# JdeRobot/slam-SDVL

Hardware: AMD Instinct MI355X
Metric: tracked frames/sec (640x480, 5-lvl pyr, ~200 feats) (higher is better)
Workload: dtype u8/f32/f64

## Files before the change

### include/sdvl_hip.h

```cpp
#ifndef SDVL_HIP_H_
#define SDVL_HIP_H_

#include <stdint.h>

#ifdef __cplusplus
extern "C" {
#endif

typedef struct sdvl_ctx sdvl_ctx;
typedef struct sdvl_frame sdvl_frame;

enum sdvl_status {
  SDVL_OK = 0,
  SDVL_ERR_INVALID = -1,
  SDVL_ERR_HIP = -2,
  SDVL_ERR_CAPACITY = -3,
  SDVL_ERR_NO_DEVICE = -4
};

#define SDVL_MAX_LEVELS 8
#define SDVL_MAX_CORNERS 6144
#define SDVL_MAX_ALIGN_FEATURES 2048
#define SDVL_CELL_KP_CAP 176
#define SDVL_MAX_CELL_SIZE 64
// ... 109 lines not shown
int sdvl_ctx_prefetch_images(sdvl_ctx *ctx, int n, const uint8_t *const *imgs, int stride, int width, int height, void *const *dev_dst);
int sdvl_ctx_prefetch_fence(sdvl_ctx *ctx, int ticket);
typedef struct sdvl_feed sdvl_feed;
int sdvl_feed_create(int device, int n_slots, sdvl_feed **out);
int sdvl_feed_destroy(sdvl_feed *f);
const char *sdvl_feed_last_error(const sdvl_feed *f);
int sdvl_feed_slot_arrived(sdvl_feed *f, int slot);
int sdvl_feed_images(sdvl_feed *f, int slot, int n, const uint8_t *const *imgs, int stride, int width, int height, void *const *dev_dst);
int sdvl_ctx_feed_acquire(sdvl_ctx *ctx, sdvl_feed *f, int slot);
int sdvl_ctx_feed_release(sdvl_ctx *ctx, sdvl_feed *f, int slot);
int sdvl_frame_set_image_device(sdvl_ctx *ctx, sdvl_frame *f, const void *dev_img, int stride);
int sdvl_frame_borrow_image_device(sdvl_ctx *ctx, sdvl_frame *f, const void *dev_img);
int sdvl_frames_own_images(sdvl_ctx *ctx, int n, sdvl_frame *const *frames);
int sdvl_pyramid_build(sdvl_ctx *ctx, int n, sdvl_frame *const *frames);
int sdvl_frame_download_level(sdvl_ctx *ctx, const sdvl_frame *f, int level, uint8_t *out, int stride);

int sdvl_fast_num_cells(int width, int height, const sdvl_detect_params *p, int *cells_per_level, int *total);
int sdvl_cell_kp_cap(int cell_size);
int64_t sdvl_detect_scratch_bytes(int width, int height, const sdvl_detect_params *p);
int sdvl_fast_cells(sdvl_ctx *ctx, int n, sdvl_frame *const *frames, const sdvl_detect_params *p, int cap,
                    sdvl_keypoint *out_kps, int32_t *out_cell_offsets);

int sdvl_detect_corners(sdvl_ctx *ctx, int n, sdvl_frame *const *frames, const sdvl_detect_params *p, int nfeatures);
int sdvl_frames_corner_counts(sdvl_ctx *ctx, int n, sdvl_frame *const *frames, int32_t *counts);
int sdvl_frame_download_corners(sdvl_ctx *ctx, sdvl_frame *f, int cap, int32_t *xyl, int *n_out);
int sdvl_retain_best(sdvl_ctx *ctx, uint32_t *packed, int len, int n_points, int cooperative, int *out_len);

int sdvl_frame_set_corners(sdvl_ctx *ctx, sdvl_frame *f, int n, const int32_t *xyl);
int sdvl_frames_set_corners(sdvl_ctx *ctx, int n, sdvl_frame *const *frames, const int32_t *counts, const int32_t *xyl);
int sdvl_frame_num_corners(const sdvl_frame *f);
int sdvl_frame_corner_capacity(const sdvl_frame *f);

int sdvl_shi_tomasi(sdvl_ctx *ctx, int n, sdvl_frame *const *frames, int cap, double *out_scores);

int sdvl_orb_describe(sdvl_ctx *ctx, int n, sdvl_frame *const *frames, int cap, uint8_t *out_desc);
int sdvl_frame_download_descriptors(sdvl_ctx *ctx, const sdvl_frame *f, int cap, uint8_t *out);
int sdvl_filter_inputs(sdvl_ctx *ctx, int n, sdvl_frame *const *frames, int cap, int32_t *xyl, double *scores, uint8_t *desc,
                       int32_t *counts);
int sdvl_filter_inputs_begin(sdvl_ctx *ctx, int n, sdvl_frame *const *frames, int cap, int with_desc);
int sdvl_filter_inputs_end(sdvl_ctx *ctx, int n, sdvl_frame *const *frames, int cap, int32_t *xyl, double *scores, uint8_t *desc,
                           int32_t *counts);
typedef struct sdvl_filtered_corner {
  int32_t index;
  int32_t x, y, level;
  int32_t score;
  int32_t pad_;
// ... 255 lines not shown
```

### slam-sdvl_amd/__init__.py

```python
import ctypes as C
import os

import numpy as np

try:
    import torch
except ImportError:
    torch = None

_HERE = os.path.dirname(os.path.abspath(__file__))
CSRC = os.path.join(_HERE, "csrc")
LIB_PATH = os.path.join(CSRC, "libsdvl_hip.so")
HOST_LIB_PATH = os.path.join(_HERE, "host", "libsdvl_host.so")

SDVL_GRAY8, SDVL_RGB8, SDVL_BGR8, SDVL_RGBA8, SDVL_BGRA8 = 0, 1, 2, 3, 4

MAX_LEVELS = 8
MAX_CORNERS = 6144

u8p = C.POINTER(C.c_uint8)
i32p = C.POINTER(C.c_int32)
f64p = C.POINTER(C.c_double)
f32p = C.POINTER(C.c_float)

# ... 68 lines not shown
class DepthParams(C.Structure):
    _fields_ = [("px_error_angle", C.c_double), ("min_depth", C.c_double), ("scale_min_dist", C.c_double),
                ("max_failed", C.c_int32), ("pad_", C.c_int32)]


class DepthOut(C.Structure):
    _fields_ = [("outcome", C.c_int32), ("n_failed", C.c_int32), ("rho", C.c_double), ("sigma2", C.c_double), ("a", C.c_double),
                ("b", C.c_double), ("cos_alpha", C.c_double), ("last_distance", C.c_double), ("position", C.c_double * 3)]


class SynthView(C.Structure):
    _fields_ = [("fx", C.c_double), ("fy", C.c_double), ("u0", C.c_double), ("v0", C.c_double),
                ("R", C.c_double * 9), ("t", C.c_double * 3), ("plane", C.c_double * 4),
                ("seed", C.c_uint32), ("frame_id", C.c_uint32), ("texture", C.c_uint32), ("reserved_", C.c_uint32),
                ("dist", C.c_double * 5)]


ABI_SYMBOLS = [
    "sdvl_ctx_create", "sdvl_ctx_destroy", "sdvl_last_error", "sdvl_ctx_synchronize", "sdvl_ctx_stream",
    "sdvl_ctx_bind_thread", "sdvl_ctx_device", "sdvl_pointer_device", "sdvl_ctx_scratch_device",
    "sdvl_ctx_timing_enable", "sdvl_ctx_timing_only", "sdvl_ctx_timing_get", "sdvl_ctx_timing_reset",
    "sdvl_frame_create", "sdvl_frame_create_many", "sdvl_frame_destroy", "sdvl_frame_upload", "sdvl_frames_upload", "sdvl_ctx_prefetch_images", "sdvl_ctx_prefetch_fence", "sdvl_frame_set_image_device", "sdvl_frame_borrow_image_device",
    "sdvl_pyramid_build", "sdvl_frame_download_level", "sdvl_fast_num_cells", "sdvl_cell_kp_cap", "sdvl_fast_cells",
    "sdvl_detect_corners", "sdvl_frames_corner_counts", "sdvl_frame_download_corners", "sdvl_retain_best",
    "sdvl_frame_set_corners", "sdvl_frames_set_corners", "sdvl_frame_num_corners", "sdvl_shi_tomasi", "sdvl_orb_describe",
    "sdvl_frame_download_descriptors", "sdvl_filter_inputs", "sdvl_filter_inputs_begin", "sdvl_filter_inputs_end", "sdvl_filter_corners_begin", "sdvl_filter_corners_end", "sdvl_orb_describe_points", "sdvl_hamming_argmin", "sdvl_image_align", "sdvl_image_align_begin", "sdvl_image_align_end", "sdvl_align_store_create", "sdvl_align_store_destroy", "sdvl_align_store_write", "sdvl_image_align_begin_stored", "sdvl_search_points", "sdvl_search_begin", "sdvl_search_slot", "sdvl_search_run", "sdvl_align_patches", "sdvl_pose_from_matches", "sdvl_search_points_filter", "sdvl_search_run_filter", "sdvl_search_run_chain", "sdvl_search_chain_end", "sdvl_frame_footprint", "sdvl_undistort", "sdvl_frames_upload_undistorted", "sdvl_convert_gray", "sdvl_frames_upload_color", "sdvl_ctx_set_wait_hook", "sdvl_ctx_wait_done", "sdvl_ctx_wait_block", "sdvl_ctx_health", "sdvl_ctx_counters",
    "sdvl_track_create", "sdvl_track_destroy", "sdvl_frame_register", "sdvl_frames_register", "sdvl_track_upload", "sdvl_track_append", "sdvl_track_align", "sdvl_track_search",
    "sdvl_track_collect", "sdvl_track_features", "sdvl_track_stats",
    "sdvl_synth_render", "sdvl_device_malloc", "sdvl_device_free", "sdvl_device_download",
    "sdvl_frames_own_images", "sdvl_feed_create", "sdvl_feed_destroy", "sdvl_feed_last_error", "sdvl_feed_slot_arrived", "sdvl_feed_images", "sdvl_ctx_feed_acquire", "sdvl_ctx_feed_release", "sdvl_frame_footprint_cap", "sdvl_ctx_set_corner_capacity", "sdvl_frame_corner_capacity", "sdvl_detect_scratch_bytes",
    "sdvl_ctx_set_wait_spin", "sdvl_ctx_fork_mark", "sdvl_ctx_fork_begin", "sdvl_ctx_fork_end", "sdvl_host_alloc_pinned", "sdvl_host_free_pinned", "sdvl_host_register", "sdvl_host_unregister",
]

_lib = None


def load_library():
    global _lib
    if _lib is None:
        if not os.path.exists(LIB_PATH):
            raise SdvlError("libsdvl_hip.so is not built (%s): run `python -c 'import __graft_entry__ as g; g.build()'`"
                            % LIB_PATH)
        lib = C.CDLL(LIB_PATH)
        lib.sdvl_last_error.restype = C.c_char_p
        lib.sdvl_last_error.argtypes = [C.c_void_p]
        lib.sdvl_ctx_stream.restype = C.c_void_p
        lib.sdvl_ctx_stream.argtypes = [C.c_void_p]
# ... 176 lines not shown

    def own_images(self, frames):
        arr = (C.c_void_p * len(frames))(*[f.h for f in frames])
        self._check(self.lib.sdvl_frames_own_images(self.h, len(frames), arr))

    def fast_cells(self, frames, dp, cap=None):
        n = len(frames)
        cpl = (C.c_int * 4)()
        tot = C.c_int()
        self._check(self.lib.sdvl_fast_num_cells(frames[0].width, frames[0].height, C.byref(dp), cpl, C.byref(tot)))
        if cap is None:
            cap = max(1, tot.value * self.lib.sdvl_cell_kp_cap(dp.cell_size))
        kps = (Keypoint * (n * cap))()
        offs = np.zeros((n, tot.value + 1), np.int32)
        arr = (C.c_void_p * n)(*[f.h for f in frames])
        self._check(self.lib.sdvl_fast_cells(self.h, n, arr, C.byref(dp), cap, kps, _ptr(offs, i32p)))
        raw = np.frombuffer(kps, dtype=np.dtype([("x", "<u2"), ("y", "<u2"), ("score", "u1"), ("level", "u1"), ("cell", "<u2")]))
        out = []
        for i in range(n):
            k = raw[i * cap: i * cap + offs[i, -1]]
            out.append((np.stack([k["x"], k["y"], k["score"], k["level"], k["cell"]], 1).astype(np.int32), offs[i].copy()))
        return out, [cpl[i] for i in range(dp.max_fast_levels)]

    def detect_corners(self, frames, dp, nfeatures=1000):
        n = len(frames)
        arr = (C.c_void_p * n)(*[f.h for f in frames])
        self._check(self.lib.sdvl_detect_corners(self.h, n, arr, C.byref(dp), nfeatures))
        counts = np.zeros(n, np.int32)
        self._check(self.lib.sdvl_frames_corner_counts(self.h, n, arr, _ptr(counts, i32p)))
        out = []
        for f, c in zip(frames, counts):
            xyl = np.zeros((max(int(c), 1), 3), np.int32)
            k = C.c_int()
            self._check(self.lib.sdvl_frame_download_corners(self.h, f.h, len(xyl), _ptr(xyl, i32p), C.byref(k)))
            out.append(xyl[:k.value].copy())
        return out

    def retain_best(self, packed, n_points, cooperative=0):
        packed = np.ascontiguousarray(packed, np.uint32).copy()
        k = C.c_int()
        self._check(self.lib.sdvl_retain_best(self.h, _ptr(packed, C.POINTER(C.c_uint32)), len(packed), int(n_points), int(cooperative),
                                              C.byref(k)))
        return packed[:k.value]

    def shi_tomasi(self, frames, cap=MAX_CORNERS):
        n = len(frames)
        out = np.zeros((n, cap), np.float64)
        arr = (C.c_void_p * n)(*[f.h for f in frames])
        self._check(self.lib.sdvl_shi_tomasi(self.h, n, arr, cap, _ptr(out, f64p)))
        return [out[i, :self.lib.sdvl_frame_num_corners(frames[i].h)].copy() for i in range(n)]
# ... 321 lines not shown
```

### slam-sdvl_amd/csrc/sdvl_detect.hip

```cpp
#include <atomic>

#include "sdvl_internal.h"
#include "sdvl_wave.h"

namespace {

constexpr int kPyrTW = 32, kPyrTH = 8;

struct PyrJob {
  const uint8_t *src;
  uint8_t *dst;
  int sw, sh, dw, dh;
};

__device__ __forceinline__ int reflect101_clamped(int p, int n) {
  if (p < 0) p = -p;
  if (p >= n) p = 2 * n - 2 - p;
  return min(max(p, 0), n - 1);
}

template <int kPyrTW, int kPyrTH>
__global__ __launch_bounds__(kPyrTW * kPyrTH / 4) void pyr_down_kernel(const PyrJob *__restrict__ jobs, int n_jobs, int gx, int gy) {
  constexpr int kThreads = kPyrTW * kPyrTH / 4;
  constexpr int kPyrSH = 2 * kPyrTH + 3;
  constexpr int kPyrSWW = kPyrTW / 2 + 2;
  constexpr int kPyrPitch = (kPyrSWW + 1) * 4;
  const auto sync = [] {
    if (kThreads == 64) wave_sync();
    else __syncthreads();
  };
  __shared__ uint32_t s_srcw[kPyrSH * (kPyrSWW + 1)];
  __shared__ __attribute__((aligned(8))) uint16_t s_h[kPyrSH][kPyrTW];
  const int id = blockIdx.x, per_frame = gx * gy;
  const int slot = id >> 3;
  const int bz = (slot / per_frame) * 8 + (id & 7);
  if (bz >= n_jobs) return;
  const int tq = slot % per_frame;
  const int by = tq / gx, bx = tq - by * gx;
  const PyrJob job = jobs[bz];
  const int tx0 = bx * kPyrTW, ty0 = by * kPyrTH;
  if (tx0 >= job.dw || ty0 >= job.dh) return;
// ... 32 lines not shown
      const int sy = reflect101_clamped(2 * ty0 - 2 + r, job.sh);
      const int wi = min(max(w0 + c, 0), words_row - 1);
      s_srcw[r * (kPyrSWW + 1) + c] = reinterpret_cast<const uint32_t *>(job.src + static_cast<size_t>(sy) * job.sw)[wi];
    }
    sync();
    if (tid < rows && (xb < 0 || xb + last_byte >= job.sw)) {
      uint8_t *row = s_bytes + tid * kPyrPitch;
      if (xb < 0) {
        row[2] = row[6];
        row[3] = row[5];
      }
      for (int b = max(2, job.sw - xb); b <= last_byte; b++) row[b] = row[max(reflect101_clamped(xb + b, job.sw) - xb, 0)];
    }
  } else {
    const int ncols = last_byte - 1;
    for (int idx = tid; idx < rows * ncols; idx += kThreads) {
      const int r = idx / ncols, c = idx - r * ncols;
      const int sy = reflect101_clamped(2 * ty0 - 2 + r, job.sh);
      const int sx = reflect101_clamped(2 * tx0 - 2 + c, job.sw);
      s_bytes[r * kPyrPitch + 2 + c] = job.src[static_cast<size_t>(sy) * job.sw + sx];
    }
  }
  sync();
  typedef unsigned short u16x2 __attribute__((ext_vector_type(2)));
  for (int idx = tid; idx < rows * (kPyrTW / 2); idx += kThreads) {
    const int r = idx / (kPyrTW / 2), xp = idx - r * (kPyrTW / 2);
    if (2 * xp < nx) {
      const uint32_t *w = &s_srcw[r * (kPyrSWW + 1) + xp];
      const uint32_t w0 = w[0], w1 = w[1], w2 = w[2];
      const uint32_t hx = __builtin_amdgcn_udot4(w1, 0x00010406u, __builtin_amdgcn_udot4(w0, 0x04010000u, 0u, false), false);
      const uint32_t hx1 = __builtin_amdgcn_udot4(w2, 0x00000001u, __builtin_amdgcn_udot4(w1, 0x04060401u, 0u, false), false);
      const uint32_t h = hx | (hx1 << 16);
      *reinterpret_cast<uint32_t *>(&s_h[r][2 * xp]) = __builtin_bit_cast(uint32_t, h);
    }
  }
  sync();
  {
    const int y = tid / (kPyrTW / 4), x = (tid % (kPyrTW / 4)) * 4;
    const int oy = ty0 + y, ox = tx0 + x;
    if (oy < job.dh && ox < job.dw) {
      u16x2 a01 = {0, 0}, a23 = {0, 0};
#pragma unroll
      for (int t = 0; t < 5; t++) {
        const unsigned short wg = (t == 0 || t == 4) ? 1 : (t == 2 ? 6 : 4);
        const u16x2 wgt = {wg, wg};
        const uint2 hv = *reinterpret_cast<const uint2 *>(&s_h[2 * y + t][x]);
        a01 += wgt * __builtin_bit_cast(u16x2, hv.x);
        a23 += wgt * __builtin_bit_cast(u16x2, hv.y);
      }
      const u16x2 half = {128, 128};
      a01 = (a01 + half) >> 8;
      a23 = (a23 + half) >> 8;
      int acc[4] = {a01.x, a01.y, a23.x, a23.y};
      uint8_t *d = job.dst + static_cast<size_t>(oy) * job.dw + ox;
      if (ox + 3 < job.dw && (reinterpret_cast<uintptr_t>(job.dst) & 3u) == 0 && (job.dw & 3) == 0) {
        __attribute__((address_space(1))) uint32_t *dstw = (__attribute__((address_space(1))) uint32_t *)job.dst;
        dstw[static_cast<uint32_t>(oy * job.dw + ox) >> 2] = __builtin_amdgcn_perm(__builtin_bit_cast(uint32_t, a23), __builtin_bit_cast(uint32_t, a01), 0x06040200u);
      } else {
#pragma unroll
        for (int k = 0; k < 4; k++)
          if (ox + k < job.dw) d[k] = static_cast<uint8_t>(acc[k]);
      }
    }
  }
}

struct FastLevels {
  int n_levels;
  int cell_begin[SDVL_MAX_LEVELS + 1];
  int wcells[SDVL_MAX_LEVELS];
  int cell_size, margin, threshold;
  int dense_num;
};

struct __attribute__((aligned(16))) CellGeo {
  uint32_t xy;
  uint32_t wh;
  int32_t level;
  int32_t pair_inv;
};

struct FastJob {
  const uint8_t *level[4];
  int lw[4], lh[4];
  uint32_t *cell_kps;
  int32_t *cell_counts;
};
// ... 995 lines not shown
    wave_sync();
    if (threadIdx.x >= kSelGroup && threadIdx.x < 2 * kSelGroup) {
      const int n = group_retain_best<kSelGroup, uint8_t>(s_v, len, n_points, gl, gr, threadIdx.x - kSelGroup, kSelGroup);
      if (threadIdx.x == kSelGroup) *out_len = n;
    }
    wave_sync();
    for (int i = threadIdx.x; i < len; i += 64) v[i] = s_v[i];
  } else if (form == 3 && len <= kSelFts) {
    for (int i = threadIdx.x; i < len; i += 64) s_v[i] = v[i];
    wave_sync();
    const int n = group_retain_best<64, uint16_t>(s_v, len, n_points, s_l, s_r, threadIdx.x, 0);
    if (threadIdx.x == 0) *out_len = n;
    wave_sync();
    for (int i = threadIdx.x; i < len; i += 64) v[i] = s_v[i];
  } else if (threadIdx.x == 0) {
    *out_len = sel_retain_best(v, len, n_points);
  }
}

}

extern "C" {

int sdvl_pyramid_build(sdvl_ctx *ctx, int n, sdvl_frame *const *frames) {
  if (!ctx || n < 0 || (n > 0 && !frames)) return SDVL_ERR_INVALID;
  if (n == 0) return SDVL_OK;
  int levels = frames[0]->v.levels;
  for (int i = 0; i < n; i++) {
    SDVL_REQUIRE(ctx, frames[i] != nullptr, "null frame");
    SDVL_REQUIRE(ctx, frames[i]->v.levels == levels && frames[i]->width == frames[0]->width && frames[i]->height == frames[0]->height,
                 "frames of one batch must share size and pyramid depth");
  }
  if (levels < 2) return SDVL_OK;
  const size_t bytes = sizeof(PyrJob) * n * (levels - 1);
  void *hs = nullptr, *dsx = nullptr;
  int rc = sdvl_stage_alloc(ctx, bytes, &hs, &dsx);
  if (rc) return rc;
  PyrJob *hj = static_cast<PyrJob *>(hs);
  for (int l = 1; l < levels; l++)
    for (int i = 0; i < n; i++) {
      const FrameView &v = frames[i]->v;
      hj[(l - 1) * n + i] = PyrJob{v.level[l - 1], v.level[l], v.lw[l - 1], v.lh[l - 1], v.lw[l], v.lh[l]};
    }
  SDVL_HIP_CHECK(ctx, sdvl_push(ctx, dsx, hj, bytes));
  for (int l = 1; l < levels; l++) {
    const FrameView &v = frames[0]->v;
    const int gx = (v.lw[l] + kPyrTW - 1) / kPyrTW, gy = (v.lh[l] + kPyrTH - 1) / kPyrTH;
    const dim3 grid = dim3(static_cast<unsigned>(gx) * gy * ((n + 7) / 8 * 8), 1, 1);
    SDVL_LAUNCH(ctx, "pyr_down", (pyr_down_kernel<kPyrTW, kPyrTH>), grid, dim3(64), static_cast<const PyrJob *>(dsx) + (l - 1) * n, n, gx, gy);
  }
  SDVL_HIP_CHECK(ctx, hipGetLastError());
  return SDVL_OK;
}

int sdvl_cell_kp_cap(int cell_size) {
  if (cell_size < 8 || cell_size > SDVL_MAX_CELL_SIZE) return 0;
  if (cell_size <= 32) return SDVL_CELL_KP_CAP;
  const int half = (cell_size - 6 + 1) / 2;
  return half * half;
}

struct DetectSlot {
  size_t counts_off, newlen_off, kps_off, spill_off, bytes;
};
static DetectSlot detect_slot_layout(int total_cells, int kp_cap, size_t spill_words) {
  DetectSlot L;
  sdvl_layout lay;
  L.counts_off = lay.take<int32_t>(static_cast<size_t>(total_cells) + 1).off;
  L.newlen_off = lay.take<int32_t>(total_cells).off;
  L.kps_off = lay.take<uint32_t>(static_cast<size_t>(kp_cap) * static_cast<size_t>(total_cells)).off;
  L.spill_off = lay.take<uint32_t>(spill_words).off;
  L.bytes = lay.bytes();
  return L;
// ... 234 lines not shown
    SDVL_HIP_CHECK(ctx, sdvl_stream_wait(ctx));
  }
  memcpy(out_cell_offsets, h_offs, offs_bytes);
  for (int i = 0; i < n; i++) {
    const int32_t *offs = h_offs + static_cast<size_t>(i) * (total_cells + 1);
    const uint32_t *src = h_kps + static_cast<size_t>(i) * cap;
    sdvl_keypoint *dst = out_kps + static_cast<size_t>(i) * cap;
    int l = 0;
    for (int c = 0; c < total_cells; c++) {
      while (l + 1 < lv.n_levels && c >= lv.cell_begin[l + 1]) l++;
      for (int k = offs[c]; k < offs[c + 1]; k++) {
        const uint32_t v = src[k];
        dst[k].x = static_cast<uint16_t>(v & 0xFFF);
        dst[k].y = static_cast<uint16_t>((v >> 12) & 0xFFF);
        dst[k].score = static_cast<uint8_t>(v >> 24);
        dst[k].level = static_cast<uint8_t>(l);
        dst[k].cell = static_cast<uint16_t>(c - lv.cell_begin[l]);
      }
    }
  }
  return SDVL_OK;
}

int sdvl_detect_corners(sdvl_ctx *ctx, int n, sdvl_frame *const *frames, const sdvl_detect_params *p, int nfeatures) {
  if (!ctx || !p || n < 0 || (n > 0 && !frames)) return SDVL_ERR_INVALID;
  if (n == 0) return SDVL_OK;
  SDVL_REQUIRE(ctx, nfeatures >= 0, "nfeatures must not be negative");
  DetectPlan pl;
  int rc = detect_plan_frames(ctx, n, frames, p, nfeatures, &pl);
  if (rc) return rc;
  const SelLevels &sl = pl.sl;
  uint8_t *scratch = nullptr;
  rc = detect_scratch(ctx, n, pl.slot, &scratch);
  if (rc) return rc;
  const size_t pack_lds = pl.pack_lds + (static_cast<size_t>(std::max(1, frames[0]->bin_cells)) * 4 + 15) / 16 * 16;
  sdvl_layout st;
  const sdvl_part<FastJob> st_fast = st.take<FastJob>(n);
  const sdvl_part<SelJob> st_sel = st.take<SelJob>(n);
  void *hst = nullptr, *dst = nullptr;
  rc = sdvl_ensure(ctx, &ctx->d_counts, &ctx->d_counts_bytes, sizeof(int32_t) * n, false);
  if (!rc) rc = sdvl_stage_alloc(ctx, st.bytes(), &hst, &dst);
  if (rc) return rc;
  ctx->detect_frames.assign(frames, frames + n);
  FastJob *hf = st_fast.in(hst);
  SelJob *hs = st_sel.in(hst);
  for (int i = 0; i < n; i++) {
    uint8_t *sb = scratch + pl.slot.bytes * i;
    hf[i] = fast_job(pl, frames[i], sb);
    memset(&hs[i], 0, sizeof(SelJob));
    for (int l = 0; l < sl.n_levels; l++) {
      hs[i].lw[l] = frames[i]->v.lw[l];
      hs[i].lh[l] = frames[i]->v.lh[l];
    }
    hs[i].cell_kps = hf[i].cell_kps;
    hs[i].cell_counts = hf[i].cell_counts;
    hs[i].cell_newlen = reinterpret_cast<int32_t *>(sb + pl.slot.newlen_off);
    hs[i].spill = reinterpret_cast<uint32_t *>(sb + pl.slot.spill_off);
    hs[i].corner_cap = frames[i]->corner_cap;
    hs[i].corner_hdr = frames[i]->v.corner_hdr;
    hs[i].bin_start = frames[i]->bin_start;
    hs[i].bin_entries = frames[i]->bin_entries;
    hs[i].bin_gw = frames[i]->bin_gw;
    hs[i].bin_cells = frames[i]->bin_cells;
    frames[i]->bins_valid = frames[i]->bin_cells > 0 ? 1 : 0;
    frames[i]->v.n_corners = -1;
    frames[i]->hdr_stale = 0;
    frames[i]->desc_valid = 0;
  }
  SDVL_HIP_CHECK(ctx, sdvl_push(ctx, dst, hst, st.bytes()));
  const FastJob *df = st_fast.cin(dst);
  const SelJob *ds = st_sel.cin(dst);
  rc = fast_launch(ctx, pl, n, frames, df);
  if (rc) return rc;
  const dim3 sel_grid(static_cast<unsigned>((n + 7) / 8 * 8 * pl.n_slices));
  if (pl.sel_form == 2)
    SDVL_LAUNCH(ctx, "select_cells", (select_cells_kernel<uint16_t, kWideCellCap, SDVL_MAX_LEVEL_CELLS, 64>), sel_grid, dim3(64), ds, sl, n);
  else if (pl.sel_form == 0)
    SDVL_LAUNCH(ctx, "select_cells", (select_cells_kernel<uint8_t, SDVL_CELL_KP_CAP, kSelMaxCells, kSelGroup>), sel_grid, dim3(64), ds, sl, n);
  else
    SDVL_LAUNCH(ctx, "select_cells", (select_cells_kernel<uint8_t, SDVL_CELL_KP_CAP, SDVL_MAX_LEVEL_CELLS, kSelGroup>), sel_grid, dim3(64), ds, sl, n);
  const bool direct = sdvl_ensure(ctx, &ctx->h_counts, &ctx->h_counts_bytes, sizeof(int32_t) * n, true) == SDVL_OK;
  if (pack_lds > (48u << 10)) {
    static std::atomic<unsigned long long> attr_devices{0};
    const int rc_a = sdvl_allow_dynamic_lds(ctx, reinterpret_cast<const void *>(select_pack_kernel), 152u << 10, &attr_devices);
    if (rc_a) return rc_a;
    SDVL_REQUIRE(ctx, pack_lds <= (152u << 10), "selection lists of this configuration do not fit a compute unit's LDS");
  }
  SDVL_LAUNCH_LDS(ctx, "select_pack", select_pack_kernel, dim3(n), dim3(256), static_cast<unsigned>(pack_lds), ds, sl, static_cast<int32_t *>(ctx->d_counts),
                  direct ? static_cast<int32_t *>(ctx->h_counts) : nullptr);
  SDVL_HIP_CHECK(ctx, hipGetLastError());
  ctx->counts_gen = ~0ull;
  if (direct) ctx->counts_gen = ctx->wait_gen;
  else if (sdvl_ensure(ctx, &ctx->h_counts, &ctx->h_counts_bytes, sizeof(int32_t) * n, true) == SDVL_OK &&
           hipMemcpyAsync(ctx->h_counts, ctx->d_counts, sizeof(int32_t) * n, hipMemcpyDeviceToHost, ctx->stream) == hipSuccess)
    ctx->counts_gen = ctx->wait_gen;
  return SDVL_OK;
}

int sdvl_frames_corner_counts(sdvl_ctx *ctx, int n, sdvl_frame *const *frames, int32_t *counts) {
  if (!ctx || n < 0 || (n > 0 && (!frames || !counts))) return SDVL_ERR_INVALID;
  if (n == 0) return SDVL_OK;
  bool all_known = true;
  for (int i = 0; i < n; i++) {
    SDVL_REQUIRE(ctx, frames[i] != nullptr, "null frame");
    if (frames[i]->v.n_corners < 0) all_known = false;
  }
  if (!all_known) {
    const size_t nd = ctx->detect_frames.size();
    int rc = sdvl_ensure(ctx, &ctx->h_out, &ctx->h_out_bytes, sizeof(int32_t) * (4 * static_cast<size_t>(n) + nd), true);
    if (rc) return rc;
    int32_t *h = static_cast<int32_t *>(ctx->h_out);
    bool batch_ok = nd > 0;
    std::vector<int> where(n, -1);
    if (batch_ok) {
      for (int i = 0; i < n && batch_ok; i++) {
        if (frames[i]->v.n_corners >= 0) continue;
        if (static_cast<size_t>(i) < nd && ctx->detect_frames[i] == frames[i]) where[i] = i;
        else {
          for (size_t k = 0; k < nd; k++)
// ... 72 lines not shown
```

### slam-sdvl_amd/host/frontend.cc

```cpp
#include "host_internal.h"

#include <algorithm>
#include <atomic>
#include <cmath>
#include <condition_variable>
#include <cstdlib>
#include <cstring>
#include <iostream>
#include <mutex>
#include <new>
#include <stdexcept>
#include <chrono>
#include <thread>

#include <sys/mman.h>

namespace sdvl {

using std::shared_ptr;
using std::vector;

static thread_local Device *g_current_device = nullptr;

static thread_local StageTimes *g_stage_times = nullptr;
// ... 404 lines not shown
    if (imgs[i].raw && frames[i]->GetCamera()->HasDistortion()) {
      const int kind = imgs[i].dev_src ? 1 : 0;
      if (!un_f[kind].empty() && (imgs[i].step != un_step[kind] || frames[i]->GetCamera() != frames[0]->GetCamera())) flush_raw(kind);
      un_step[kind] = imgs[i].step;
      un_f[kind].push_back(devs[i]);
      un_i[kind].push_back(imgs[i].dev_src ? imgs[i].dev_src : static_cast<const void *>(imgs[i].data));
      continue;
    }
    if (imgs[i].dev_src && imgs[i].step == imgs[i].cols && imgs[i].borrow) {
      dev->Check(sdvl_frame_borrow_image_device(dev->ctx(), devs[i], imgs[i].dev_src), "sdvl_frame_borrow_image_device");
      frames[i]->SetImageTransient(imgs[i].transient);
    } else {
      if (!up_f.empty() && (imgs[i].step != up_step || frames[i]->GetWidth() != frames[0]->GetWidth() || frames[i]->GetHeight() != frames[0]->GetHeight()))
        flush();
      up_step = imgs[i].step;
      up_f.push_back(devs[i]);
      up_i.push_back(imgs[i].dev_src ? static_cast<const uint8_t *>(imgs[i].dev_src) : imgs[i].data);
    }
  }
  flush();
  flush_raw(0);
  flush_raw(1);
  flush_color();
  dev->Check(sdvl_pyramid_build(dev->ctx(), n, devs.data()), "sdvl_pyramid_build");
  if (!corners) return;
  const sdvl_detect_params dp = DetectParams();
  clk.reset(new StageClock(ST_FAST));
  dev->Check(sdvl_detect_corners(dev->ctx(), n, devs.data(), &dp, nfeatures), "sdvl_detect_corners");
  clk.reset(new StageClock(ST_CORNERS_ORB));
}
}

Frame::Frame(Camera *camera, ORBDetector *detector, const Image &img, bool corners) {
  InitCommon(camera, detector, img.cols, img.rows);
  BuildFrames({this}, {dev_}, {img}, corners, Config::NumFeatures());
  corners_on_host_ = !corners;
}

void Frame::CreateBatch(Camera *camera, ORBDetector *detector, const vector<Image> &imgs, bool corners, int nfeatures,
                        vector<shared_ptr<Frame>> *out, const std::function<void(int, std::function<void(int)>)> *pfor) {
  const int n = static_cast<int>(imgs.size());
  vector<Frame *> raw(n);
  vector<sdvl_frame *> devs(n);
  out->clear();
  std::unique_ptr<StageClock> clk(new StageClock(ST_PRELUDE));
  for (int i = 0; i < n; i++) {
    shared_ptr<Frame> f(new Frame());
    f->InitCommon(camera, detector, imgs[i].cols, imgs[i].rows);
    raw[i] = f.get();
    devs[i] = f->dev_;
    f->corners_on_host_ = !corners;
// ... 914 lines not shown
```

### slam-sdvl_amd/host/standalone.cc

```cpp
#include "sdvl_host.h"
#include "host_internal.h"

#include <algorithm>
#include <atomic>
#include <cmath>
#include <condition_variable>
#include <cstdlib>
#include <cstring>
#include <iostream>
#include <mutex>
#include <new>
#include <stdexcept>
#include <chrono>
#include <thread>

#include <sys/mman.h>

namespace sdvl {

using std::shared_ptr;
using std::vector;

Camera::Camera() {
  const CameraParameters &p = Config::GetCameraParameters();
// ... 1127 lines not shown
    prm.pad_ = 0;
    const sdvl_camera cam = camera.abi();
    const bool fork_detect = !detected_ahead && !detected_now && B <= 4;
    if (fork_detect) dev_->Check(sdvl_ctx_fork_mark(dev_->ctx()), "sdvl_ctx_fork_mark");
    dev_->Check(sdvl_track_align(dev_->ctx(), track_, R, tr_jobs_.data(), tr_rank_.data(), tr_rand_.data(), &cam, &prm), "sdvl_track_align");
    if (fork_detect) {
      dev_->Check(sdvl_ctx_fork_begin(dev_->ctx()), "sdvl_ctx_fork_begin");
      try {
        Frame::DetectBatch(frames, Config::NumFeatures());
      } catch (...) {
        (void)sdvl_ctx_fork_end(dev_->ctx());
        throw;
      }
      dev_->Check(sdvl_ctx_fork_end(dev_->ctx()), "sdvl_ctx_fork_end");
    } else if (!detected_ahead && !detected_now) {
      Frame::DetectBatch(frames, Config::NumFeatures());
    }
    clk.reset(new StageClock(ST_SEARCH));
    dev_->Check(sdvl_track_search(dev_->ctx(), track_), "sdvl_track_search");
    if (!next_imgs_.empty() && R == B && static_cast<int>(next_imgs_.size()) == B) {
      bool device_images = true;
      for (const Image &im : next_imgs_) device_images = device_images && im.dev_src != nullptr && !im.transient;
      if (device_images) {
        Frame::CreateBatch(&camera, &trk_[0]->orb_detector_, next_imgs_, false, Config::NumFeatures(), &ahead_frames_, &pfor);
        Frame::DetectBatch(ahead_frames_, Config::NumFeatures());
        ahead_src_.clear();
        for (const Image &im : next_imgs_) ahead_src_.push_back(im.dev_src);
      }
    }
    tr_res_.resize(R);
    dev_->Check(sdvl_track_collect(dev_->ctx(), track_, R, tr_res_.data()), "sdvl_track_collect");

    clk.reset(new StageClock(ST_FINISH));
    for (int k = 0; k < R; k++)
      if (tr_res_[k].status != 0) throw std::runtime_error("sdvl_track: a table capacity was exceeded on the device");
    ParallelFor(R, [&](int k) {
      const int i = run[k];
      SDVL &t = *trk_[i];
      FrameStats &st = stats[i];
      const sdvl_track_result &r = tr_res_[k];
      SDVL::TrackState &ts = t.track_;
      st.align_meas = r.align_meas;
      st.align_iters = r.align_iters;
      st.align_features = r.n_features;
      st.search_requests = r.n_requests;
      st.lk_iters = r.lk_iters;
      st.n_corners = r.n_corners;
      t.current_frame_->SetPose(SE3::FromArray(r.pose));
// ... 605 lines not shown
```

Measured before the change: 457,300.

## Fuse pyramid levels in pairs and merge pyramid build with detection staging

```diff
diff --git a/include/sdvl_hip.h b/include/sdvl_hip.h
--- a/include/sdvl_hip.h
+++ b/include/sdvl_hip.h
@@ -155,6 +155,7 @@
                     sdvl_keypoint *out_kps, int32_t *out_cell_offsets);
 
 int sdvl_detect_corners(sdvl_ctx *ctx, int n, sdvl_frame *const *frames, const sdvl_detect_params *p, int nfeatures);
+int sdvl_pyramid_detect(sdvl_ctx *ctx, int n, sdvl_frame *const *frames, const sdvl_detect_params *p, int nfeatures);
 int sdvl_frames_corner_counts(sdvl_ctx *ctx, int n, sdvl_frame *const *frames, int32_t *counts);
 int sdvl_frame_download_corners(sdvl_ctx *ctx, sdvl_frame *f, int cap, int32_t *xyl, int *n_out);
 int sdvl_retain_best(sdvl_ctx *ctx, uint32_t *packed, int len, int n_points, int cooperative, int *out_len);
diff --git a/slam-sdvl_amd/__init__.py b/slam-sdvl_amd/__init__.py
--- a/slam-sdvl_amd/__init__.py
+++ b/slam-sdvl_amd/__init__.py
@@ -114,7 +114,7 @@
     "sdvl_ctx_timing_enable", "sdvl_ctx_timing_only", "sdvl_ctx_timing_get", "sdvl_ctx_timing_reset",
     "sdvl_frame_create", "sdvl_frame_create_many", "sdvl_frame_destroy", "sdvl_frame_upload", "sdvl_frames_upload", "sdvl_ctx_prefetch_images", "sdvl_ctx_prefetch_fence", "sdvl_frame_set_image_device", "sdvl_frame_borrow_image_device",
     "sdvl_pyramid_build", "sdvl_frame_download_level", "sdvl_fast_num_cells", "sdvl_cell_kp_cap", "sdvl_fast_cells",
-    "sdvl_detect_corners", "sdvl_frames_corner_counts", "sdvl_frame_download_corners", "sdvl_retain_best",
+    "sdvl_detect_corners", "sdvl_pyramid_detect", "sdvl_frames_corner_counts", "sdvl_frame_download_corners", "sdvl_retain_best",
     "sdvl_frame_set_corners", "sdvl_frames_set_corners", "sdvl_frame_num_corners", "sdvl_shi_tomasi", "sdvl_orb_describe",
     "sdvl_frame_download_descriptors", "sdvl_filter_inputs", "sdvl_filter_inputs_begin", "sdvl_filter_inputs_end", "sdvl_filter_corners_begin", "sdvl_filter_corners_end", "sdvl_orb_describe_points", "sdvl_hamming_argmin", "sdvl_image_align", "sdvl_image_align_begin", "sdvl_image_align_end", "sdvl_align_store_create", "sdvl_align_store_destroy", "sdvl_align_store_write", "sdvl_image_align_begin_stored", "sdvl_search_points", "sdvl_search_begin", "sdvl_search_slot", "sdvl_search_run", "sdvl_align_patches", "sdvl_pose_from_matches", "sdvl_search_points_filter", "sdvl_search_run_filter", "sdvl_search_run_chain", "sdvl_search_chain_end", "sdvl_frame_footprint", "sdvl_undistort", "sdvl_frames_upload_undistorted", "sdvl_convert_gray", "sdvl_frames_upload_color", "sdvl_ctx_set_wait_hook", "sdvl_ctx_wait_done", "sdvl_ctx_wait_block", "sdvl_ctx_health", "sdvl_ctx_counters",
     "sdvl_track_create", "sdvl_track_destroy", "sdvl_frame_register", "sdvl_frames_register", "sdvl_track_upload", "sdvl_track_append", "sdvl_track_align", "sdvl_track_search",
@@ -337,10 +337,10 @@
             out.append((np.stack([k["x"], k["y"], k["score"], k["level"], k["cell"]], 1).astype(np.int32), offs[i].copy()))
         return out, [cpl[i] for i in range(dp.max_fast_levels)]
 
-    def detect_corners(self, frames, dp, nfeatures=1000):
+    def detect_corners(self, frames, dp, nfeatures=1000, pyramid=False):
         n = len(frames)
         arr = (C.c_void_p * n)(*[f.h for f in frames])
-        self._check(self.lib.sdvl_detect_corners(self.h, n, arr, C.byref(dp), nfeatures))
+        self._check((self.lib.sdvl_pyramid_detect if pyramid else self.lib.sdvl_detect_corners)(self.h, n, arr, C.byref(dp), nfeatures))
         counts = np.zeros(n, np.int32)
         self._check(self.lib.sdvl_frames_corner_counts(self.h, n, arr, _ptr(counts, i32p)))
         out = []
diff --git a/slam-sdvl_amd/csrc/sdvl_detect.hip b/slam-sdvl_amd/csrc/sdvl_detect.hip
--- a/slam-sdvl_amd/csrc/sdvl_detect.hip
+++ b/slam-sdvl_amd/csrc/sdvl_detect.hip
@@ -17,6 +17,52 @@
   if (p < 0) p = -p;
   if (p >= n) p = 2 * n - 2 - p;
   return min(max(p, 0), n - 1);
+}
+
+template <int kTW, int kThreads, int kPitchW>
+__device__ __forceinline__ void pyr_horizontal(const uint32_t *s_srcw, uint16_t (*s_h)[kTW], int rows, int nx, int tid) {
+  for (int idx = tid; idx < rows * (kTW / 2); idx += kThreads) {
+    const int r = idx / (kTW / 2), xp = idx - r * (kTW / 2);
+    if (2 * xp < nx) {
+      const uint32_t *w = &s_srcw[r * kPitchW + xp];
+      const uint32_t w0 = w[0], w1 = w[1], w2 = w[2];
+      const uint32_t hx = __builtin_amdgcn_udot4(w1, 0x00010406u, __builtin_amdgcn_udot4(w0, 0x04010000u, 0u, false), false);
+      const uint32_t hx1 = __builtin_amdgcn_udot4(w2, 0x00000001u, __builtin_amdgcn_udot4(w1, 0x04060401u, 0u, false), false);
+      *reinterpret_cast<uint32_t *>(&s_h[r][2 * xp]) = hx | (hx1 << 16);
+    }
+  }
+}
+
+typedef unsigned short pyr_u16x2 __attribute__((ext_vector_type(2)));
+
+template <int kTW>
+__device__ __forceinline__ void pyr_vertical_store(const uint16_t (*s_h)[kTW], uint8_t *dst, int dw, int dh, int tx0, int ty0, int tid) {
+  const int y = tid / (kTW / 4), x = (tid % (kTW / 4)) * 4;
+  const int oy = ty0 + y, ox = tx0 + x;
+  if (oy < dh && ox < dw) {
+    pyr_u16x2 a01 = {0, 0}, a23 = {0, 0};
+#pragma unroll
+    for (int t = 0; t < 5; t++) {
+      const unsigned short wg = (t == 0 || t == 4) ? 1 : (t == 2 ? 6 : 4);
+      const pyr_u16x2 wgt = {wg, wg};
+      const uint2 hv = *reinterpret_cast<const uint2 *>(&s_h[2 * y + t][x]);
+      a01 += wgt * __builtin_bit_cast(pyr_u16x2, hv.x);
+      a23 += wgt * __builtin_bit_cast(pyr_u16x2, hv.y);
+    }
+    const pyr_u16x2 half = {128, 128};
+    a01 = (a01 + half) >> 8;
+    a23 = (a23 + half) >> 8;
+    int acc[4] = {a01.x, a01.y, a23.x, a23.y};
+    uint8_t *d = dst + static_cast<size_t>(oy) * dw + ox;
+    if (ox + 3 < dw && (reinterpret_cast<uintptr_t>(dst) & 3u) == 0 && (dw & 3) == 0) {
+      __attribute__((address_space(1))) uint32_t *dstw = (__attribute__((address_space(1))) uint32_t *)dst;
+      dstw[static_cast<uint32_t>(oy * dw + ox) >> 2] = __builtin_amdgcn_perm(__builtin_bit_cast(uint32_t, a23), __builtin_bit_cast(uint32_t, a01), 0x06040200u);
+    } else {
+#pragma unroll
+      for (int k = 0; k < 4; k++)
+        if (ox + k < dw) d[k] = static_cast<uint8_t>(acc[k]);
+    }
+  }
 }
 
 template <int kPyrTW, int kPyrTH>
@@ -95,47 +141,179 @@
     }
   }
   sync();
-  typedef unsigned short u16x2 __attribute__((ext_vector_type(2)));
-  for (int idx = tid; idx < rows * (kPyrTW / 2); idx += kThreads) {
-    const int r = idx / (kPyrTW / 2), xp = idx - r * (kPyrTW / 2);
-    if (2 * xp < nx) {
-      const uint32_t *w = &s_srcw[r * (kPyrSWW + 1) + xp];
-      const uint32_t w0 = w[0], w1 = w[1], w2 = w[2];
-      const uint32_t hx = __builtin_amdgcn_udot4(w1, 0x00010406u, __builtin_amdgcn_udot4(w0, 0x04010000u, 0u, false), false);
-      const uint32_t hx1 = __builtin_amdgcn_udot4(w2, 0x00000001u, __builtin_amdgcn_udot4(w1, 0x04060401u, 0u, false), false);
-      const uint32_t h = hx | (hx1 << 16);
-      *reinterpret_cast<uint32_t *>(&s_h[r][2 * xp]) = __builtin_bit_cast(uint32_t, h);
-    }
-  }
+  pyr_horizontal<kPyrTW, kThreads, kPyrSWW + 1>(s_srcw, s_h, rows, nx, tid);
   sync();
+  pyr_vertical_store<kPyrTW>(s_h, job.dst, job.dw, job.dh, tx0, ty0, tid);
+}
+
+constexpr int kPairMW = 2 * kPyrTW + 3, kPairMH = 2 * kPyrTH + 3;
+constexpr int kPairMPitch = kPyrTW / 2 + 2;
+constexpr int kPairSH = 2 * kPairMH + 3;
+constexpr int kPairSPitch = 36;
+
+struct PyrPairJob {
+  const uint8_t *src;
+  uint8_t *mid, *dst;
+  int sw, sh, mw, mh, dw, dh;
+};
+
+__global__ __launch_bounds__(64) void pyr_down_pair_kernel(const PyrPairJob *__restrict__ jobs, int n_jobs, int gx, int gy) {
+  __shared__ __attribute__((aligned(16))) uint32_t s_src_pad[4 + (kPairSH + 1) * kPairSPitch];
+  uint32_t *const s_src = s_src_pad + 4;
+  __shared__ __attribute__((aligned(16))) uint32_t s_mid[kPairMH * kPairMPitch];
+  __shared__ __attribute__((aligned(8))) uint16_t s_h[kPairMH][kPyrTW];
+  const int id = blockIdx.x, per_frame = gx * gy;
+  const int slot = id >> 3;
+  const int bz = (slot / per_frame) * 8 + (id & 7);
+  if (bz >= n_jobs) return;
+  const int tq = slot % per_frame;
+  const int by = tq / gx, bx = tq - by * gx;
+  const PyrPairJob job = jobs[bz];
+  const int tx0 = bx * kPyrTW, ty0 = by * kPyrTH;
+  if (2 * tx0 >= job.mw || 2 * ty0 >= job.mh) return;
+  const int tid = threadIdx.x;
+  const int px0 = 2 * tx0 - 2, py0 = 2 * ty0 - 2;
+  const int xb = 4 * tx0 - 8, yb = 4 * ty0 - 6;
+  const int ncx = min(kPairMW, job.mw - px0), ncy = min(kPairMH, job.mh - py0);
+  const int rows = 2 * ncy + 3, last_byte = 2 * ncx + 4;
+  uint8_t *s_bytes = reinterpret_cast<uint8_t *>(s_src);
+  if ((job.sw & 3) == 0 && (reinterpret_cast<uintptr_t>(job.src) & 3u) == 0) {
+    const int words_row = job.sw >> 2, w0 = xb >> 2;
+    const int nwords = last_byte / 4 + 1;
+    constexpr int kRowLanes = (kPairSPitch + 3) / 4, kRowsPerRound = 64 / kRowLanes, kRounds = (kPairSH + kRowsPerRound - 1) / kRowsPerRound;
+    if (words_row >= 4) {
+      const int lr = tid / kRowLanes, lq = tid - lr * kRowLanes;
+      const int first = w0 + 4 * lq;
+      const int s = min(max(first, 0), words_row - 4);
+      const int col0 = s - w0;
+      if (lr < kRowsPerRound && 4 * lq < nwords) {
+        const __attribute__((address_space(1))) uint32_t *srcw = (const __attribute__((address_space(1))) uint32_t *)job.src;
+        uint32_t v[kRounds][4];
+#pragma unroll
+        for (int k = 0; k < kRounds; k++) {
+          const int sy = reflect101_clamped(yb + lr + k * kRowsPerRound, job.sh);
+          const __attribute__((address_space(1))) uint32_t *pw = srcw + static_cast<uint32_t>(sy * words_row + s);
+#pragma unroll
+          for (int j = 0; j < 4; j++) v[k][j] = pw[j];
+        }
+#pragma unroll
+        for (int k = 0; k < kRounds; k++) {
+          uint32_t *dst = &s_src[(lr + k * kRowsPerRound) * kPairSPitch + col0];
+#pragma unroll
+          for (int j = 0; j < 4; j++) dst[j] = v[k][j];
+        }
+      }
+    } else
+    for (int idx = tid; idx < rows * kPairSPitch; idx += 64) {
+      const int r = idx / kPairSPitch, c = idx - r * kPairSPitch;
+      if (c >= nwords) continue;
+      const int sy = reflect101_clamped(yb + r, job.sh);
+      const int wi = min(max(w0 + c, 0), words_row - 1);
+      s_src[idx] = reinterpret_cast<const uint32_t *>(job.src + static_cast<size_t>(sy) * job.sw)[wi];
+    }
+    wave_sync();
+    if (tid < rows && (xb < 0 || xb + last_byte >= job.sw)) {
+      uint8_t *row = s_bytes + tid * (kPairSPitch * 4);
+      for (int b = 2; b < min(-xb, last_byte + 1); b++) row[b] = row[max(reflect101_clamped(xb + b, job.sw) - xb, 0)];
+      for (int b = max(2, job.sw - xb); b <= last_byte; b++) row[b] = row[max(reflect101_clamped(xb + b, job.sw) - xb, 0)];
+    }
+  } else {
+    const int ncols = last_byte - 1;
+    for (int idx = tid; idx < rows * ncols; idx += 64) {
+      const int r = idx / ncols, c = idx - r * ncols;
+      const int sy = reflect101_clamped(yb + r, job.sh);
+      const int sx = reflect101_clamped(xb + 2 + c, job.sw);
+      s_bytes[r * (kPairSPitch * 4) + 2 + c] = job.src[static_cast<size_t>(sy) * job.sw + sx];
+    }
+  }
+  wave_sync();
   {
-    const int y = tid / (kPyrTW / 4), x = (tid % (kPyrTW / 4)) * 4;
-    const int oy = ty0 + y, ox = tx0 + x;
-    if (oy < job.dh && ox < job.dw) {
-      u16x2 a01 = {0, 0}, a23 = {0, 0};
-#pragma unroll
-      for (int t = 0; t < 5; t++) {
-        const unsigned short wg = (t == 0 || t == 4) ? 1 : (t == 2 ? 6 : 4);
-        const u16x2 wgt = {wg, wg};
-        const uint2 hv = *reinterpret_cast<const uint2 *>(&s_h[2 * y + t][x]);
-        a01 += wgt * __builtin_bit_cast(u16x2, hv.x);
-        a23 += wgt * __builtin_bit_cast(u16x2, hv.y);
-      }
-      const u16x2 half = {128, 128};
-      a01 = (a01 + half) >> 8;
-      a23 = (a23 + half) >> 8;
-      int acc[4] = {a01.x, a01.y, a23.x, a23.y};
-      uint8_t *d = job.dst + static_cast<size_t>(oy) * job.dw + ox;
-      if (ox + 3 < job.dw && (reinterpret_cast<uintptr_t>(job.dst) & 3u) == 0 && (job.dw & 3) == 0) {
-        __attribute__((address_space(1))) uint32_t *dstw = (__attribute__((address_space(1))) uint32_t *)job.dst;
-        dstw[static_cast<uint32_t>(oy * job.dw + ox) >> 2] = __builtin_amdgcn_perm(__builtin_bit_cast(uint32_t, a23), __builtin_bit_cast(uint32_t, a01), 0x06040200u);
+    constexpr int kQuads = (kPairMW + 3) / 4;
+    const int g = tid / kQuads, k = tid - g * kQuads;
+    const int r0 = g == 0 ? 0 : (g == 1 ? 7 : 13);
+    const int r1 = g > 2 ? 0 : min(g == 0 ? 7 : (g == 1 ? 13 : kPairMH), ncy);
+    const auto hsum = [&](int row) {
+      const uint2 *p = reinterpret_cast<const uint2 *>(&s_src[row * kPairSPitch + 2 * k]);
+      const uint2 a = p[0], b = p[1];
+      const uint32_t h0 = __builtin_amdgcn_udot4(a.y, 0x00010406u, __builtin_amdgcn_udot4(a.x, 0x04010000u, 0u, false), false);
+      const uint32_t h1 = __builtin_amdgcn_udot4(b.x, 0x00000001u, __builtin_amdgcn_udot4(a.y, 0x04060401u, 0u, false), false);
+      const uint32_t h2 = __builtin_amdgcn_udot4(b.x, 0x00010406u, __builtin_amdgcn_udot4(a.y, 0x04010000u, 0u, false), false);
+      const uint32_t h3 = __builtin_amdgcn_udot4(b.y, 0x00000001u, __builtin_amdgcn_udot4(b.x, 0x04060401u, 0u, false), false);
+      return make_uint2(h0 | (h1 << 16), h2 | (h3 << 16));
+    };
+    if (r0 < r1) {
+      uint2 ha = hsum(2 * r0), hb = hsum(2 * r0 + 1), hc = hsum(2 * r0 + 2);
+      uint16_t *mid16 = reinterpret_cast<uint16_t *>(s_mid);
+      for (int r = r0; r < r1; r++) {
+        const uint2 hd = hsum(2 * r + 3), he = hsum(2 * r + 4);
+        const pyr_u16x2 one4 = {4, 4}, one6 = {6, 6}, half = {128, 128};
+        pyr_u16x2 a01 = __builtin_bit_cast(pyr_u16x2, ha.x) + __builtin_bit_cast(pyr_u16x2, he.x) + half;
+        pyr_u16x2 a23 = __builtin_bit_cast(pyr_u16x2, ha.y) + __builtin_bit_cast(pyr_u16x2, he.y) + half;
+        a01 += one4 * (__builtin_bit_cast(pyr_u16x2, hb.x) + __builtin_bit_cast(pyr_u16x2, hd.x)) + one6 * __builtin_bit_cast(pyr_u16x2, hc.x);
+        a23 += one4 * (__builtin_bit_cast(pyr_u16x2, hb.y) + __builtin_bit_cast(pyr_u16x2, hd.y)) + one6 * __builtin_bit_cast(pyr_u16x2, hc.y);
+        a01 >>= 8;
+        a23 >>= 8;
+        uint16_t *m = mid16 + r * (kPairMPitch * 2) + 2 * k + 1;
+        m[0] = static_cast<uint16_t>(a01.x | (a01.y << 8));
+        m[1] = static_cast<uint16_t>(a23.x | (a23.y << 8));
+        ha = hc;
+        hb = hd;
+        hc = he;
+      }
+    }
+  }
+  wave_sync();
+  uint8_t *m_bytes = reinterpret_cast<uint8_t *>(s_mid);
+  const int cr = job.mw - px0, rr = job.mh - py0;
+  const bool fix_r = job.mw == 2 * job.dw && cr < kPairMW, fix_b = job.mh == 2 * job.dh && rr < kPairMH;
+  if (px0 < 0 || fix_r || py0 < 0 || fix_b) {
+    if (tid < kPairMH) {
+      uint8_t *row = m_bytes + tid * (kPairMPitch * 4) + 2;
+      if (px0 < 0) {
+        row[0] = row[reflect101_clamped(-2, job.mw) + 2];
+        row[1] = row[reflect101_clamped(-1, job.mw) + 2];
+      }
+      if (fix_r) row[cr] = row[cr - 2];
+    }
+    wave_sync();
+    if (tid < kPairMPitch) {
+      uint32_t *col = s_mid + tid;
+      if (py0 < 0) {
+        col[0] = col[(reflect101_clamped(-2, job.mh) + 2) * kPairMPitch];
+        col[kPairMPitch] = col[(reflect101_clamped(-1, job.mh) + 2) * kPairMPitch];
+      }
+      if (fix_b) col[rr * kPairMPitch] = col[(rr - 2) * kPairMPitch];
+    }
+    wave_sync();
+  }
+  {
+    const int y = tid >> 2, q = tid & 3;
+    const int oy = 2 * ty0 + y, ox = 2 * tx0 + 16 * q;
+    if (oy < job.mh && ox < job.mw) {
+      const uint32_t *w = &s_mid[(y + 2) * kPairMPitch + 1 + 4 * q];
+      const uint32_t v[4] = {w[0], w[1], w[2], w[3]};
+      typedef __attribute__((address_space(1))) uint8_t gbyte;
+      gbyte *d = (gbyte *)job.mid + static_cast<uint32_t>(oy * job.mw + ox);
+      if ((job.mw & 3) == 0 && (reinterpret_cast<uintptr_t>(job.mid) & 15u) == 0) {
+        typedef unsigned int u32x4 __attribute__((ext_vector_type(4)));
+        if ((job.mw & 15) == 0) *(__attribute__((address_space(1))) u32x4 *)d = u32x4{v[0], v[1], v[2], v[3]};
+        else {
+#pragma unroll
+          for (int j = 0; j < 4; j++)
+            if (ox + 4 * j < job.mw) ((__attribute__((address_space(1))) uint32_t *)d)[j] = v[j];
+        }
       } else {
 #pragma unroll
-        for (int k = 0; k < 4; k++)
-          if (ox + k < job.dw) d[k] = static_cast<uint8_t>(acc[k]);
-      }
-    }
-  }
+        for (int j = 0; j < 16; j++)
+          if (ox + j < job.mw) d[j] = static_cast<uint8_t>(v[j >> 2] >> (8 * (j & 3)));
+      }
+    }
+  }
+  if (tx0 >= job.dw || ty0 >= job.dh) return;
+  const int nx = min(kPyrTW, job.dw - tx0), ny = min(kPyrTH, job.dh - ty0);
+  pyr_horizontal<kPyrTW, 64, kPairMPitch>(s_mid, s_h, 2 * ny + 3, nx, tid);
+  wave_sync();
+  pyr_vertical_store<kPyrTW>(s_h, job.dst, job.dw, job.dh, tx0, ty0, tid);
 }
 
 struct FastLevels {
@@ -1177,33 +1355,64 @@
 
 extern "C" {
 
-int sdvl_pyramid_build(sdvl_ctx *ctx, int n, sdvl_frame *const *frames) {
-  if (!ctx || n < 0 || (n > 0 && !frames)) return SDVL_ERR_INVALID;
-  if (n == 0) return SDVL_OK;
-  int levels = frames[0]->v.levels;
+struct PyrPlan {
+  int n_pairs, single;
+  sdvl_part<PyrPairJob> pair[(SDVL_MAX_LEVELS - 1) / 2];
+  sdvl_part<PyrJob> one;
+};
+
+static int pyr_plan(sdvl_ctx *ctx, int n, sdvl_frame *const *frames, sdvl_layout *st, PyrPlan *pp) {
+  const int levels = frames[0] ? frames[0]->v.levels : 0;
   for (int i = 0; i < n; i++) {
     SDVL_REQUIRE(ctx, frames[i] != nullptr, "null frame");
     SDVL_REQUIRE(ctx, frames[i]->v.levels == levels && frames[i]->width == frames[0]->width && frames[i]->height == frames[0]->height,
                  "frames of one batch must share size and pyramid depth");
   }
-  if (levels < 2) return SDVL_OK;
-  const size_t bytes = sizeof(PyrJob) * n * (levels - 1);
-  void *hs = nullptr, *dsx = nullptr;
-  int rc = sdvl_stage_alloc(ctx, bytes, &hs, &dsx);
+  pp->n_pairs = (levels - 1) / 2;
+  pp->single = levels >= 2 && (levels - 1) % 2 ? levels - 1 : 0;
+  for (int k = 0; k < pp->n_pairs; k++) pp->pair[k] = st->take<PyrPairJob>(n);
+  pp->one = st->take<PyrJob>(pp->single ? n : 0);
+  return SDVL_OK;
+}
+
+static void pyr_fill(const PyrPlan &pp, int n, sdvl_frame *const *frames, void *hst) {
+  for (int i = 0; i < n; i++) {
+    const FrameView &v = frames[i]->v;
+    for (int k = 0; k < pp.n_pairs; k++) {
+      const int l = 2 * k;
+      pp.pair[k].in(hst)[i] = PyrPairJob{v.level[l], v.level[l + 1], v.level[l + 2], v.lw[l], v.lh[l], v.lw[l + 1], v.lh[l + 1], v.lw[l + 2], v.lh[l + 2]};
+    }
+    if (const int l = pp.single) pp.one.in(hst)[i] = PyrJob{v.level[l - 1], v.level[l], v.lw[l - 1], v.lh[l - 1], v.lw[l], v.lh[l]};
+  }
+}
+
+static void pyr_launch(sdvl_ctx *ctx, const PyrPlan &pp, int n, sdvl_frame *const *frames, const void *dst) {
+  const FrameView &v = frames[0]->v;
+  const unsigned slots = static_cast<unsigned>((n + 7) / 8 * 8);
+  for (int k = 0; k < pp.n_pairs; k++) {
+    const int gx = (v.lw[2 * k + 1] + 2 * kPyrTW - 1) / (2 * kPyrTW), gy = (v.lh[2 * k + 1] + 2 * kPyrTH - 1) / (2 * kPyrTH);
+    SDVL_LAUNCH(ctx, "pyr_down", pyr_down_pair_kernel, dim3(gx * gy * slots), dim3(64), pp.pair[k].cin(dst), n, gx, gy);
+  }
+  if (const int l = pp.single) {
+    const int gx = (v.lw[l] + kPyrTW - 1) / kPyrTW, gy = (v.lh[l] + kPyrTH - 1) / kPyrTH;
+    SDVL_LAUNCH(ctx, "pyr_down", (pyr_down_kernel<kPyrTW, kPyrTH>), dim3(gx * gy * slots), dim3(64), pp.one.cin(dst), n, gx, gy);
+  }
+}
+
+int sdvl_pyramid_build(sdvl_ctx *ctx, int n, sdvl_frame *const *frames) {
+  if (!ctx || n < 0 || (n > 0 && !frames)) return SDVL_ERR_INVALID;
+  if (n == 0) return SDVL_OK;
+  sdvl_layout st;
+  PyrPlan pp;
+  int rc = pyr_plan(ctx, n, frames, &st, &pp);
   if (rc) return rc;
-  PyrJob *hj = static_cast<PyrJob *>(hs);
-  for (int l = 1; l < levels; l++)
-    for (int i = 0; i < n; i++) {
-      const FrameView &v = frames[i]->v;
-      hj[(l - 1) * n + i] = PyrJob{v.level[l - 1], v.level[l], v.lw[l - 1], v.lh[l - 1], v.lw[l], v.lh[l]};
-    }
-  SDVL_HIP_CHECK(ctx, sdvl_push(ctx, dsx, hj, bytes));
-  for (int l = 1; l < levels; l++) {
-    const FrameView &v = frames[0]->v;
-    const int gx = (v.lw[l] + kPyrTW - 1) / kPyrTW, gy = (v.lh[l] + kPyrTH - 1) / kPyrTH;
-    const dim3 grid = dim3(static_cast<unsigned>(gx) * gy * ((n + 7) / 8 * 8), 1, 1);
-    SDVL_LAUNCH(ctx, "pyr_down", (pyr_down_kernel<kPyrTW, kPyrTH>), grid, dim3(64), static_cast<const PyrJob *>(dsx) + (l - 1) * n, n, gx, gy);
-  }
+  if (frames[0]->v.levels < 2) return SDVL_OK;
+  void *hst = nullptr, *dst = nullptr;
+  rc = sdvl_stage_alloc(ctx, st.bytes(), &hst, &dst);
+  if (rc) return rc;
+  pyr_fill(pp, n, frames, hst);
+  SDVL_HIP_CHECK(ctx, sdvl_push(ctx, dst, hst, st.bytes()));
+  pyr_launch(ctx, pp, n, frames, dst);
   SDVL_HIP_CHECK(ctx, hipGetLastError());
   return SDVL_OK;
 }
@@ -1484,30 +1693,34 @@
   return SDVL_OK;
 }
 
-int sdvl_detect_corners(sdvl_ctx *ctx, int n, sdvl_frame *const *frames, const sdvl_detect_params *p, int nfeatures) {
-  if (!ctx || !p || n < 0 || (n > 0 && !frames)) return SDVL_ERR_INVALID;
-  if (n == 0) return SDVL_OK;
+struct DetectBatch {
+  DetectPlan pl;
+  uint8_t *scratch;
+  size_t pack_lds;
+  sdvl_part<FastJob> fast;
+  sdvl_part<SelJob> sel;
+};
+
+static int detect_prepare(sdvl_ctx *ctx, int n, sdvl_frame *const *frames, const sdvl_detect_params *p, int nfeatures, sdvl_layout *st, DetectBatch *b) {
   SDVL_REQUIRE(ctx, nfeatures >= 0, "nfeatures must not be negative");
-  DetectPlan pl;
-  int rc = detect_plan_frames(ctx, n, frames, p, nfeatures, &pl);
+  int rc = detect_plan_frames(ctx, n, frames, p, nfeatures, &b->pl);
   if (rc) return rc;
+  rc = detect_scratch(ctx, n, b->pl.slot, &b->scratch);
+  if (rc) return rc;
+  b->pack_lds = b->pl.pack_lds + (static_cast<size_t>(std::max(1, frames[0]->bin_cells)) * 4 + 15) / 16 * 16;
+  b->fast = st->take<FastJob>(n);
+  b->sel = st->take<SelJob>(n);
+  return sdvl_ensure(ctx, &ctx->d_counts, &ctx->d_counts_bytes, sizeof(int32_t) * n, false);
+}
+
+static void detect_fill(sdvl_ctx *ctx, const DetectBatch &b, int n, sdvl_frame *const *frames, void *hst) {
+  const DetectPlan &pl = b.pl;
   const SelLevels &sl = pl.sl;
-  uint8_t *scratch = nullptr;
-  rc = detect_scratch(ctx, n, pl.slot, &scratch);
-  if (rc) return rc;
-  const size_t pack_lds = pl.pack_lds + (static_cast<size_t>(std::max(1, frames[0]->bin_cells)) * 4 + 15) / 16 * 16;
-  sdvl_layout st;
-  const sdvl_part<FastJob> st_fast = st.take<FastJob>(n);
-  const sdvl_part<SelJob> st_sel = st.take<SelJob>(n);
-  void *hst = nullptr, *dst = nullptr;
-  rc = sdvl_ensure(ctx, &ctx->d_counts, &ctx->d_counts_bytes, sizeof(int32_t) * n, false);
-  if (!rc) rc = sdvl_stage_alloc(ctx, st.bytes(), &hst, &dst);
-  if (rc) return rc;
   ctx->detect_frames.assign(frames, frames + n);
-  FastJob *hf = st_fast.in(hst);
-  SelJob *hs = st_sel.in(hst);
+  FastJob *hf = b.fast.in(hst);
+  SelJob *hs = b.sel.in(hst);
   for (int i = 0; i < n; i++) {
-    uint8_t *sb = scratch + pl.slot.bytes * i;
+    uint8_t *sb = b.scratch + pl.slot.bytes * i;
     hf[i] = fast_job(pl, frames[i], sb);
     memset(&hs[i], 0, sizeof(SelJob));
     for (int l = 0; l < sl.n_levels; l++) {
@@ -1529,10 +1742,15 @@
     frames[i]->hdr_stale = 0;
     frames[i]->desc_valid = 0;
   }
-  SDVL_HIP_CHECK(ctx, sdvl_push(ctx, dst, hst, st.bytes()));
-  const FastJob *df = st_fast.cin(dst);
-  const SelJob *ds = st_sel.cin(dst);
-  rc = fast_launch(ctx, pl, n, frames, df);
+}
+
+static int detect_launch(sdvl_ctx *ctx, const DetectBatch &b, int n, sdvl_frame *const *frames, const void *dst) {
+  const DetectPlan &pl = b.pl;
+  const SelLevels &sl = pl.sl;
+  const size_t pack_lds = b.pack_lds;
+  const FastJob *df = b.fast.cin(dst);
+  const SelJob *ds = b.sel.cin(dst);
+  int rc = fast_launch(ctx, pl, n, frames, df);
   if (rc) return rc;
   const dim3 sel_grid(static_cast<unsigned>((n + 7) / 8 * 8 * pl.n_slices));
   if (pl.sel_form == 2)
@@ -1557,6 +1775,40 @@
            hipMemcpyAsync(ctx->h_counts, ctx->d_counts, sizeof(int32_t) * n, hipMemcpyDeviceToHost, ctx->stream) == hipSuccess)
     ctx->counts_gen = ctx->wait_gen;
   return SDVL_OK;
+}
+
+int sdvl_detect_corners(sdvl_ctx *ctx, int n, sdvl_frame *const *frames, const sdvl_detect_params *p, int nfeatures) {
+  if (!ctx || !p || n < 0 || (n > 0 && !frames)) return SDVL_ERR_INVALID;
+  if (n == 0) return SDVL_OK;
+  sdvl_layout st;
+  DetectBatch b;
+  int rc = detect_prepare(ctx, n, frames, p, nfeatures, &st, &b);
+  if (rc) return rc;
+  void *hst = nullptr, *dst = nullptr;
+  rc = sdvl_stage_alloc(ctx, st.bytes(), &hst, &dst);
+  if (rc) return rc;
+  detect_fill(ctx, b, n, frames, hst);
+  SDVL_HIP_CHECK(ctx, sdvl_push(ctx, dst, hst, st.bytes()));
+  return detect_launch(ctx, b, n, frames, dst);
+}
+
+int sdvl_pyramid_detect(sdvl_ctx *ctx, int n, sdvl_frame *const *frames, const sdvl_detect_params *p, int nfeatures) {
+  if (!ctx || !p || n < 0 || (n > 0 && !frames)) return SDVL_ERR_INVALID;
+  if (n == 0) return SDVL_OK;
+  sdvl_layout st;
+  PyrPlan pp;
+  DetectBatch b;
+  int rc = pyr_plan(ctx, n, frames, &st, &pp);
+  if (!rc) rc = detect_prepare(ctx, n, frames, p, nfeatures, &st, &b);
+  if (rc) return rc;
+  void *hst = nullptr, *dst = nullptr;
+  rc = sdvl_stage_alloc(ctx, st.bytes(), &hst, &dst);
+  if (rc) return rc;
+  pyr_fill(pp, n, frames, hst);
+  detect_fill(ctx, b, n, frames, hst);
+  SDVL_HIP_CHECK(ctx, sdvl_push(ctx, dst, hst, st.bytes()));
+  pyr_launch(ctx, pp, n, frames, dst);
+  return detect_launch(ctx, b, n, frames, dst);
 }
 
 int sdvl_frames_corner_counts(sdvl_ctx *ctx, int n, sdvl_frame *const *frames, int32_t *counts) {
diff --git a/slam-sdvl_amd/host/frontend.cc b/slam-sdvl_amd/host/frontend.cc
--- a/slam-sdvl_amd/host/frontend.cc
+++ b/slam-sdvl_amd/host/frontend.cc
@@ -450,11 +450,13 @@
   flush_raw(0);
   flush_raw(1);
   flush_color();
-  dev->Check(sdvl_pyramid_build(dev->ctx(), n, devs.data()), "sdvl_pyramid_build");
-  if (!corners) return;
+  if (!corners) {
+    dev->Check(sdvl_pyramid_build(dev->ctx(), n, devs.data()), "sdvl_pyramid_build");
+    return;
+  }
   const sdvl_detect_params dp = DetectParams();
   clk.reset(new StageClock(ST_FAST));
-  dev->Check(sdvl_detect_corners(dev->ctx(), n, devs.data(), &dp, nfeatures), "sdvl_detect_corners");
+  dev->Check(sdvl_pyramid_detect(dev->ctx(), n, devs.data(), &dp, nfeatures), "sdvl_pyramid_detect");
   clk.reset(new StageClock(ST_CORNERS_ORB));
 }
 }
diff --git a/slam-sdvl_amd/host/standalone.cc b/slam-sdvl_amd/host/standalone.cc
--- a/slam-sdvl_amd/host/standalone.cc
+++ b/slam-sdvl_amd/host/standalone.cc
@@ -1173,8 +1173,7 @@
       bool device_images = true;
       for (const Image &im : next_imgs_) device_images = device_images && im.dev_src != nullptr && !im.transient;
       if (device_images) {
-        Frame::CreateBatch(&camera, &trk_[0]->orb_detector_, next_imgs_, false, Config::NumFeatures(), &ahead_frames_, &pfor);
-        Frame::DetectBatch(ahead_frames_, Config::NumFeatures());
+        Frame::CreateBatch(&camera, &trk_[0]->orb_detector_, next_imgs_, true, Config::NumFeatures(), &ahead_frames_, &pfor);
         ahead_src_.clear();
         for (const Image &im : next_imgs_) ahead_src_.push_back(im.dev_src);
       }
```

After: 438,700. 0.959x the previous value.
